# yatpor/bpc_baseline

Hardware: NVIDIA B200
Metric: matched+triangulated scenes/s with the ROI crops of every match (crops/s alongside) (higher is better)
Workload: dtype f64 geometry / u8+f32 crops

## Files before the change

### bpc_baseline_b200/_lib.py

```python
from __future__ import annotations

import ctypes as C
import os

HERE = os.path.dirname(os.path.abspath(__file__))
LIB_PATH = os.environ.get('BPC_LIB') or os.path.join(HERE, 'libbpc_b200.so')

_p = C.c_void_p
_i = C.c_int
_f = C.c_float
_sz = C.c_size_t

SIGNATURES = {
    'bpc_abi_version': (_i, []),
    'bpc_error_string': (C.c_char_p, [_i]),
    'bpc_launch_count': (C.c_ulonglong, []),
    'bpc_fundamental': (_i, [_p, _p, _i, _p, _p]),
    'bpc_cost_tensor': (_i, [_p, _p, _p, _i, _i, _p, _p]),
    'bpc_match_objects': (_i, [_p, _i, _i, _i, _i, _f, _p, _p, _p]),
    'bpc_match_workspace_bytes': (_sz, [_i, _i]),
    'bpc_match_triangulate': (_i, [_p, _p, _p, _p, _i, _i, _f, _i, C.c_double, _p, _p, _p, _p, _p, _p, _p, _sz, _p]),
    'bpc_pack_records_bytes': (_sz, [_i, _i]),
    'bpc_pack_records': (_i, [_p, _p, _p, _p, _p, _p, _i, _i, _i, _p, _p]),
    'bpc_triangulate': (_i, [_p, _p, _i, _p, _p]),
    'bpc_projection': (_i, [_p, _p, _i, _p, _p]),
    'bpc_reprojection_error': (_i, [_p, _p, _p, _i, _p, _p]),
    'bpc_epipolar_error': (_i, [_p, _p, _p, _i, _p, _p]),
    'bpc_epipolar_error_full': (_i, [_p, _p, _i, _p, _p]),
    'bpc_triangulate_views': (_i, [_p, _p, _i, _i, _p, _p]),
    'bpc_box_centers': (_i, [_p, _i, _p, _p]),
    'bpc_detections_from_yolo': (_i, [_p, _p, _p, _p, _i, _i, _f, _i, _p, _p, _p, _p]),
    'bpc_build_rois': (_i, [_p, _p, _p, _p, _i, _i, _i, _p, _p, _p]),
    'bpc_train_rois': (_i, [_p, _p, _p, _p, _i, _i, _i, _p, _p]),
    'bpc_roi_crop_workspace_bytes': (_sz, [_i, _i]),
    'bpc_roi_crop': (_i, [_p, _i, _i, _i, _p, _i, _p, _i, _i, _p, _i, _p, _p, _p, _p, _sz, _p]),
    'bpc_roi_crop_u8': (_i, [_p, _i, _i, _i, _p, _i, _p, _i, _i, _p, _p, _p, _p, _sz, _p]),
    'bpc_roi_crop_bf16': (_i, [_p, _i, _i, _i, _p, _i, _p, _i, _i, _p, _i, _p, _p, _p, _p, _sz, _p]),
    'bpc_normalise_lut': (_i, [_p, _p, _p, _p]),
    'bpc_crops_normalise': (_i, [_p, _p, _i, _i, _i, _p, _p, _p]),
    'bpc_color_jitter': (_i, [_p, _i, _i, _p, _p, _i, _p, _p, _p]),
}

_lib = None
ABI_VERSION = 2


class BpcError(RuntimeError):
    pass


def load():
    global _lib
    if _lib is not None:
        return _lib
    if not os.path.exists(LIB_PATH):
        raise BpcError(f'{LIB_PATH} not found: build it with `python -m bpc_baseline_b200.build` '
                       '(or __graft_entry__.build()); there is no CPU fallback')
    lib = C.CDLL(LIB_PATH)
    for name, (res, args) in SIGNATURES.items():
        fn = getattr(lib, name)
        fn.restype = res
        fn.argtypes = args
    if lib.bpc_abi_version() != ABI_VERSION:
        raise BpcError(f'ABI version mismatch: library {lib.bpc_abi_version()}, binding {ABI_VERSION}')
    _lib = lib
    return lib


def check(code: int, what: str):
    if code != 0:
        msg = load().bpc_error_string(code).decode()
        raise BpcError(f'{what} failed with code {code}: {msg}')


def launch_count() -> int:
    return int(load().bpc_launch_count())
```

### bpc_baseline_b200/batched.py

```python
from __future__ import annotations

import ctypes as C
from dataclasses import dataclass
from typing import Optional, Sequence

import numpy as np
import torch

from . import _lib

MEAN = (0.485, 0.456, 0.406)
STD = (0.229, 0.224, 0.225)


def _chk(t: torch.Tensor, dtype, name: str, ndim: Optional[int] = None):
    if not isinstance(t, torch.Tensor):
        raise TypeError(f'{name}: expected a torch.Tensor, got {type(t).__name__}')
    if not t.is_cuda:
        raise RuntimeError(f'{name}: must be a CUDA tensor (no CPU fallback)')
    if t.dtype != dtype:
        raise RuntimeError(f'{name}: dtype {t.dtype}, expected {dtype}')
    if not t.is_contiguous():
        raise RuntimeError(f'{name}: must be contiguous')
    if ndim is not None and t.dim() != ndim:
# ... 216 lines not shown


def epipolar_error_full(F: torch.Tensor, pts: torch.Tensor) -> torch.Tensor:
    _chk(F, torch.float64, 'F', 4); _chk(pts, torch.float64, 'pts', 3)
    n = F.shape[0]
    if tuple(F.shape) != (n, 3, 3, 3) or tuple(pts.shape) != (n, 3, 2):
        raise RuntimeError('expected F [n,3,3,3] and pts [n,3,2]')
    e = torch.empty((n,), dtype=torch.float64, device=F.device)
    with torch.cuda.device(F.device):
        _lib.check(_lib.load().bpc_epipolar_error_full(_p(F), _p(pts), n, _p(e), _stream(F.device)), 'bpc_epipolar_error_full')
    return e


def triangulate_views(P: torch.Tensor, pts: torch.Tensor) -> torch.Tensor:
    _chk(P, torch.float64, 'P', 4); _chk(pts, torch.float64, 'pts', 3)
    n, V = P.shape[0], P.shape[1]
    if tuple(P.shape) != (n, V, 3, 4) or tuple(pts.shape) != (n, V, 2) or not 2 <= V <= 8:
        raise RuntimeError('expected P [n,V,3,4] and pts [n,V,2] with 2 <= V <= 8')
    X = torch.empty((n, 3), dtype=torch.float64, device=P.device)
    with torch.cuda.device(P.device):
        _lib.check(_lib.load().bpc_triangulate_views(_p(P), _p(pts), n, V, _p(X), _stream(P.device)), 'bpc_triangulate_views')
    return X


def build_rois(boxes: torch.Tensor, idx: torch.Tensor, n: torch.Tensor, image_of_scene: torch.Tensor,
               rois: Optional[torch.Tensor] = None) -> tuple[torch.Tensor, torch.Tensor]:
    _chk(boxes, torch.int32, 'boxes', 4); _chk(idx, torch.int32, 'idx', 3); _chk(n, torch.int32, 'n', 1)
    _chk(image_of_scene, torch.int32, 'image_of_scene', 2)
    S, _, D, _ = boxes.shape
    K = idx.shape[1]
    dev = boxes.device
    if rois is None:
        rois = torch.empty((S * K * 3, 5), dtype=torch.int32, device=dev)
    else:
        _chk(rois, torch.int32, 'rois', 2)
        if rois.shape[0] < S * K * 3 or rois.shape[1] != 5:
            raise RuntimeError('rois must be int32 [>= S*Kmax*3, 5]')
    offs = torch.empty((S + 1,), dtype=torch.int32, device=dev)
    with torch.cuda.device(dev):
        _lib.check(_lib.load().bpc_build_rois(_p(boxes), _p(idx), _p(n), _p(image_of_scene), S, D, K, _p(offs), _p(rois),
                                              _stream(dev)), 'bpc_build_rois')
    return rois, offs


_LUT_CACHE: dict = {}


def normalise_lut(device, mean: Sequence[float] = MEAN, std: Sequence[float] = STD) -> torch.Tensor:
    device = torch.device(device)
    key = (device.index if device.index is not None else torch.cuda.current_device(), tuple(mean), tuple(std))
    if key not in _LUT_CACHE:
        lut = torch.empty((3, 256), dtype=torch.float32, device=device)
        m = (C.c_float * 3)(*[float(np.float32(v)) for v in mean])
        s = (C.c_float * 3)(*[float(np.float32(v)) for v in std])
        with torch.cuda.device(device):
            _lib.check(_lib.load().bpc_normalise_lut(m, s, _p(lut), _stream(device)), 'bpc_normalise_lut')
        _LUT_CACHE[key] = lut
    return _LUT_CACHE[key]


_WS_CACHE: dict = {}
MAX_ROIS_PER_LAUNCH = 32768
MAX_TARGET = 1024
MAX_ROI_WIDTH = 8192


def _crop_workspace(dev, R: int, T: int) -> torch.Tensor:
    need = int(_lib.load().bpc_roi_crop_workspace_bytes(int(R), int(T)))
    key = (dev.index if dev.index is not None else torch.cuda.current_device(), int(torch.cuda.current_stream(dev).cuda_stream))
    ws = _WS_CACHE.get(key)
    if ws is None or ws.numel() < need:
        ws = torch.empty((max(need, 1 << 16),), dtype=torch.uint8, device=dev)
        _WS_CACHE[key] = ws
    return ws


def _chk_status(status, R: int) -> None:
    if status is not None:
        _chk(status, torch.int32, 'status', 1)
        if status.shape[0] < R:
            raise RuntimeError('status must hold one int32 per ROI')


def _crop_args(images, rois, T, fill):
    _chk(images, torch.uint8, 'images', 4); _chk(rois, torch.int32, 'rois', 2)
    B, H, W, ch = images.shape
    if ch != 3 or rois.shape[1] != 5:
        raise RuntimeError('images must be [B,H,W,3] and rois [R,5]')
    if not 1 <= int(T) <= MAX_TARGET:
        raise RuntimeError(f'target size must be in 1..{MAX_TARGET}')
    f = (C.c_uint8 * 3)(*[int(v) for v in fill])
    return B, H, W, rois.shape[0], f


def roi_crop(images: torch.Tensor, rois: torch.Tensor, T: int = 256, fill=(255, 255, 255), swap_rb: bool = True,
             lut: Optional[torch.Tensor] = None, n_rois: Optional[torch.Tensor] = None, roi_first: int = 0,
             out: Optional[torch.Tensor] = None, status: Optional[torch.Tensor] = None) -> torch.Tensor:
    B, H, W, R, f = _crop_args(images, rois, T, fill)
    dev = images.device
    if lut is None:
        lut = normalise_lut(dev)
    _chk_lut(lut, dev)
    if out is None:
        out = torch.empty((R, 3, T, T), dtype=torch.float32, device=dev)
    else:
        _chk(out, torch.float32, 'out', 4)
        if out.shape[0] < R or tuple(out.shape[1:]) != (3, T, T):
            raise RuntimeError('out must be [>=R,3,T,T]')
        _chk_device(out, dev, 'out')
    _chk_status(status, R)
    if n_rois is not None:
        _chk(n_rois, torch.int32, 'n_rois')
    ws = _crop_workspace(dev, min(R, MAX_ROIS_PER_LAUNCH), T)
    with torch.cuda.device(dev):
        for lo in range(0, R, MAX_ROIS_PER_LAUNCH):
            r = min(MAX_ROIS_PER_LAUNCH, R - lo)
            _lib.check(_lib.load().bpc_roi_crop(_p(images), B, H, W, _p(rois[lo:lo + r]), r, _p(n_rois), int(roi_first) + lo, int(T),
                                                f, int(bool(swap_rb)), _p(lut), _p(out[lo:lo + r]),
                                                _p(status[lo:lo + r]) if status is not None else None,
                                                _p(ws), ws.numel(), _stream(dev)), 'bpc_roi_crop')
    return out


def roi_crop_bf16(images: torch.Tensor, rois: torch.Tensor, T: int = 256, fill=(255, 255, 255), swap_rb: bool = True,
                  lut: Optional[torch.Tensor] = None, n_rois: Optional[torch.Tensor] = None, roi_first: int = 0,
                  out: Optional[torch.Tensor] = None, status: Optional[torch.Tensor] = None) -> torch.Tensor:
    B, H, W, R, f = _crop_args(images, rois, T, fill)
    dev = images.device
    if lut is None:
        lut = normalise_lut(dev)
    _chk_lut(lut, dev)
    if out is None:
        out = torch.empty((R, 3, T, T), dtype=torch.bfloat16, device=dev, memory_format=torch.channels_last)
    else:
        if out.dtype != torch.bfloat16 or not out.is_cuda or out.dim() != 4 or out.shape[0] < R or tuple(out.shape[1:]) != (3, T, T) \
                or not out.is_contiguous(memory_format=torch.channels_last):
            raise RuntimeError('out must be a channels_last bfloat16 CUDA tensor [>=R,3,T,T]')
        _chk_device(out, dev, 'out')
    _chk_status(status, R)
    if n_rois is not None:
        _chk(n_rois, torch.int32, 'n_rois')
    ws = _crop_workspace(dev, min(R, MAX_ROIS_PER_LAUNCH), T)
    with torch.cuda.device(dev):
        for lo in range(0, R, MAX_ROIS_PER_LAUNCH):
            r = min(MAX_ROIS_PER_LAUNCH, R - lo)
            _lib.check(_lib.load().bpc_roi_crop_bf16(_p(images), B, H, W, _p(rois[lo:lo + r]), r, _p(n_rois), int(roi_first) + lo, int(T),
                                                     f, int(bool(swap_rb)), _p(lut), out[lo:lo + r].data_ptr(),
                                                     _p(status[lo:lo + r]) if status is not None else None,
                                                     _p(ws), ws.numel(), _stream(dev)), 'bpc_roi_crop_bf16')
    return out


def roi_crop_u8(images: torch.Tensor, rois: torch.Tensor, T: int = 256, fill=(255, 255, 255),
                   n_rois: Optional[torch.Tensor] = None, roi_first: int = 0, out: Optional[torch.Tensor] = None,
                status: Optional[torch.Tensor] = None) -> torch.Tensor:
    B, H, W, R, f = _crop_args(images, rois, T, fill)
    dev = images.device
    if out is None:
        out = torch.empty((R, T, T, 3), dtype=torch.uint8, device=dev)
    else:
        _chk(out, torch.uint8, 'out', 4)
        if out.shape[0] < R or tuple(out.shape[1:]) != (T, T, 3):
            raise RuntimeError('out must be uint8 [>=R,T,T,3]')
        _chk_device(out, dev, 'out')
    _chk_status(status, R)
    if n_rois is not None:
        _chk(n_rois, torch.int32, 'n_rois')
    ws = _crop_workspace(dev, min(R, MAX_ROIS_PER_LAUNCH), T)
    with torch.cuda.device(dev):
        for lo in range(0, R, MAX_ROIS_PER_LAUNCH):
            r = min(MAX_ROIS_PER_LAUNCH, R - lo)
            _lib.check(_lib.load().bpc_roi_crop_u8(_p(images), B, H, W, _p(rois[lo:lo + r]), r, _p(n_rois), int(roi_first) + lo, int(T),
                                                   f, _p(out[lo:lo + r]), _p(status[lo:lo + r]) if status is not None else None,
                                                   _p(ws), ws.numel(), _stream(dev)), 'bpc_roi_crop_u8')
    return out


def crops_normalise(sources: Sequence[torch.Tensor], T: int, swap_rb: bool = True, lut: Optional[torch.Tensor] = None,
                    out: Optional[torch.Tensor] = None, device=None) -> torch.Tensor:
    if not 1 <= len(sources) <= 16:
        raise RuntimeError('1..16 sources')
    for s in sources:
        _chk(s, torch.uint8, 'sources[*]', 4)
        if tuple(s.shape[1:]) != (T, T, 3):
            raise RuntimeError('every source must be uint8 [n,T,T,3]')
    dev = torch.device(device) if device is not None else sources[0].device
    if dev.type == 'cuda' and dev.index is None:
        dev = torch.device('cuda', torch.cuda.current_device())
    if lut is None:
        lut = normalise_lut(dev)
    _chk_lut(lut, dev)
    total = sum(int(s.shape[0]) for s in sources)
    if out is None:
        out = torch.empty((total, 3, T, T), dtype=torch.float32, device=dev)
    else:
        _chk(out, torch.float32, 'out', 4)
        if out.shape[0] < total or tuple(out.shape[1:]) != (3, T, T):
            raise RuntimeError('out must be [>=sum(n_s),3,T,T]')
        _chk_device(out, dev, 'out')
    ptrs = (C.c_void_p * len(sources))(*[s.data_ptr() if s.shape[0] else None for s in sources])
    counts = (C.c_int32 * len(sources))(*[int(s.shape[0]) for s in sources])
    with torch.cuda.device(dev):
        _lib.check(_lib.load().bpc_crops_normalise(ptrs, counts, len(sources), int(T), int(bool(swap_rb)), _p(lut), _p(out),
                                                   _stream(dev)), 'bpc_crops_normalise')
    return out


def color_jitter(canvases: torch.Tensor, order: torch.Tensor, factors: torch.Tensor, swap_rb: bool = False,
                 lut: Optional[torch.Tensor] = None, out: Optional[torch.Tensor] = None) -> torch.Tensor:
    _chk(canvases, torch.uint8, 'canvases', 4); _chk(order, torch.int32, 'order', 2); _chk(factors, torch.float32, 'factors', 2)
    n, T = canvases.shape[0], canvases.shape[1]
    if tuple(canvases.shape[1:]) != (T, T, 3) or tuple(order.shape) != (n, 4) or tuple(factors.shape) != (n, 4):
        raise RuntimeError('expected canvases [n,T,T,3], order [n,4] and factors [n,4]')
    if not 1 <= T <= MAX_TARGET:
        raise RuntimeError(f'target size must be in 1..{MAX_TARGET}')
    dev = canvases.device
    if order.device != dev or factors.device != dev:
        raise RuntimeError('canvases, order and factors must be on the same device')
    if lut is None:
        lut = normalise_lut(dev)
    _chk_lut(lut, dev)
    if out is None:
        out = torch.empty((n, 3, T, T), dtype=torch.float32, device=dev)
    else:
        _chk(out, torch.float32, 'out', 4)
        if out.shape[0] < n or tuple(out.shape[1:]) != (3, T, T):
            raise RuntimeError('out must be [>=n,3,T,T]')
        _chk_device(out, dev, 'out')
    with torch.cuda.device(dev):
        _lib.check(_lib.load().bpc_color_jitter(_p(canvases), n, T, _p(order), _p(factors), int(bool(swap_rb)), _p(lut), _p(out),
                                                _stream(dev)), 'bpc_color_jitter')
    return out


def train_rois(xywh: torch.Tensor, W: int, H: int, image: Optional[torch.Tensor] = None, scale: Optional[torch.Tensor] = None,
               shift: Optional[torch.Tensor] = None) -> torch.Tensor:
    _chk(xywh, torch.int32, 'xywh', 2)
    n = xywh.shape[0]
    if xywh.shape[1] != 4:
        raise RuntimeError('xywh must be [n,4]')
    if image is not None:
        _chk(image, torch.int32, 'image', 1)
    if scale is not None:
        _chk(scale, torch.float64, 'scale', 1)
    if shift is not None:
        _chk(shift, torch.int32, 'shift', 2)
        if scale is None:
            raise RuntimeError('shift needs scale (the reference draws both, data_utils.py:257-263)')
    for t, name in ((image, 'image'), (scale, 'scale'), (shift, 'shift')):
        if t is not None and t.shape[0] != n:
            raise RuntimeError(f'{name}: first dimension must be {n}')
    dev = xywh.device
    rois = torch.empty((n, 5), dtype=torch.int32, device=dev)
    with torch.cuda.device(dev):
        _lib.check(_lib.load().bpc_train_rois(_p(xywh), _p(image), _p(scale), _p(shift), n, int(W), int(H), _p(rois),
                                              _stream(dev)), 'bpc_train_rois')
    return rois
# ... 1 lines not shown
```

### bpc_baseline_b200/csrc/crop.cu

```cuda
#include <mutex>
#include <type_traits>

#include "crop_common.cuh"

namespace bpc {

#ifndef BPC_PREP_THREADS
#define BPC_PREP_THREADS 128
#endif
constexpr int PREP_THREADS = BPC_PREP_THREADS;

__device__ void src_row_records(float2* ysrc, int cap, const RoiGeom& g, int maxtaps, int tid, int* bad) {
    const int hpad = min(cap, ((g.h + STREAM_ROWS - 1) / STREAM_ROWS) * STREAM_ROWS + STREAM_ROWS);
    if (g.h + STREAM_ROWS > cap) *bad = 1;
    for (int s = tid; s < hpad; s += PREP_THREADS) ysrc[s] = make_float2(0.f, 0.f);
    __syncthreads();
    for (int d = tid; d < g.new_h && !*bad; d += PREP_THREADS) {
        int ys, yn, fl; float bf, bm, bl;
        area_taps(d, g.scale_y, g.h, ys, yn, bf, bm, bl, fl);
        const int prev_last = d > 0 ? area_last_tap(d - 1, g.scale_y, g.h) : -1;
        if (yn < 1 || yn > maxtaps || ys < prev_last || ys + yn > g.h) { *bad = 1; break; }
        for (int t = 0; t < yn; ++t) {
            const int s = ys + t;
            const bool shared_first = (t == 0 && s == prev_last);
// ... 774 lines not shown
                        const int32_t* __restrict__ glist, const int32_t* __restrict__ gcount, int T, int nbands,
                        uchar4 fill, int swap_rb, const float* __restrict__ lut_g, float* __restrict__ outf, uint8_t* __restrict__ outb) {
    extern __shared__ __align__(16) unsigned char raw[];
    __shared__ RoiGeom g;
    __shared__ YDesc yd[CROP_BAND];
    __shared__ float lut[OUT_U8 ? 1 : 3 * LUT_STRIDE];
    const int tid = threadIdx.x, nth = blockDim.x;
    const long long items = (long long)(*gcount) * nbands;
    if (blockIdx.x >= items) return;
    if (!OUT_U8)
        for (int e = tid; e < 768; e += nth) lut[(e >> 8) * LUT_STRIDE + (e & 255)] = lut_g[e];
    __syncthreads();
    Out<OUT_U8, BF16> out;
    out_init(out, outf, outb, lut, T, swap_rb, fill);
    for (long long item = blockIdx.x; item < items; item += gridDim.x) {
        const int roi = glist[item / nbands], band = (int)(item % nbands);
        __syncthreads();
        if (tid == 0) g = geom[roi];
        __syncthreads();
        crop_generic_band<OUT_U8, BF16>(raw, yd, out, g, roi, band, images, B, H, W, T, tid, nth);
    }
}

__global__ void bpc_lut_kernel(float m0, float m1, float m2, float s0, float s1, float s2, float* __restrict__ lut) {
    const int t = blockIdx.x * blockDim.x + threadIdx.x;
    if (t >= 768) return;
    const int c = t >> 8, v = t & 255;
    const float mean = c == 0 ? m0 : (c == 1 ? m1 : m2);
    const float sd = c == 0 ? s0 : (c == 1 ? s1 : s2);
    lut[t] = __fdiv_rn(__fsub_rn(__fdiv_rn((float)v, 255.f), mean), sd);
}

static int tensor_maps(const uint8_t* images, int B, int H, int W, bool aligned, TmapSet* out) {
    typedef CUresult (*EncodeFn)(CUtensorMap*, CUtensorMapDataType, cuuint32_t, void*, const cuuint64_t*, const cuuint64_t*,
                                 const cuuint32_t*, const cuuint32_t*, CUtensorMapInterleave, CUtensorMapSwizzle,
                                 CUtensorMapL2promotion, CUtensorMapFloatOOBfill);
    static std::mutex mu;
    static TmapSet cached;
    static const uint8_t* k_images = nullptr;
    static int k_B = 0, k_H = 0, k_W = 0, k_dev = -1;
    static EncodeFn encode = nullptr;
    std::lock_guard<std::mutex> lock(mu);
    if (!aligned) { memset(out, 0, sizeof(TmapSet)); return BPC_OK; }
    int dev = 0;
    cudaGetDevice(&dev);
    if (images == k_images && B == k_B && H == k_H && W == k_W && dev == k_dev) { *out = cached; return BPC_OK; }
    if (!encode) {
        cudaDriverEntryPointQueryResult q;
        void* fnp = nullptr;
        cudaError_t e = cudaGetDriverEntryPoint("cuTensorMapEncodeTiled", &fnp, cudaEnableDefault, &q);
        if (e != cudaSuccess) return (int)e;
        if (q != cudaDriverEntryPointSuccess || !fnp) return (int)cudaErrorNotSupported;
        encode = (EncodeFn)fnp;
    }
    const cuuint64_t gdim[2] = {(cuuint64_t)W * 3 / 4, (cuuint64_t)B * H};
    const cuuint64_t gstride[1] = {(cuuint64_t)W * 3};
    const cuuint32_t estr[2] = {1, 1};
    for (int i = 0; i < N_TMAPS; ++i) {
        const int pitch = i < 13 ? 64 + 32 * i : 512 + 64 * (i - 13);
        const cuuint32_t box[2] = {(cuuint32_t)pitch / 4, (cuuint32_t)tmap_rows(pitch)};
        const CUresult r = encode(&cached.m[i], CU_TENSOR_MAP_DATA_TYPE_UINT32, 2, (void*)images, gdim, gstride, box, estr,
                                  CU_TENSOR_MAP_INTERLEAVE_NONE, CU_TENSOR_MAP_SWIZZLE_NONE, BPC_L2_PROMO,
                                  CU_TENSOR_MAP_FLOAT_OOB_FILL_NONE);
        if (r != CUDA_SUCCESS) { k_images = nullptr; return (int)cudaErrorInvalidValue; }
    }
    for (int i = 0; i < N_TMAPS8; ++i) {
        const int pitch = 64 + 32 * i;
        const cuuint32_t box[2] = {(cuuint32_t)pitch / 4, (cuuint32_t)STREAM_ROWS};
        const CUresult r = encode(&cached.m8[i], CU_TENSOR_MAP_DATA_TYPE_UINT32, 2, (void*)images, gdim, gstride, box, estr,
                                  CU_TENSOR_MAP_INTERLEAVE_NONE, CU_TENSOR_MAP_SWIZZLE_NONE, BPC_L2_PROMO,
                                  CU_TENSOR_MAP_FLOAT_OOB_FILL_NONE);
        if (r != CUDA_SUCCESS) { k_images = nullptr; return (int)cudaErrorInvalidValue; }
    }
    k_images = images; k_B = B; k_H = H; k_W = W; k_dev = dev;
    *out = cached;
    return BPC_OK;
}

static size_t ws_off_xdesc(int R) { return (((size_t)R * sizeof(RoiGeom)) + 15) & ~(size_t)15; }
static size_t ws_off_ydesc(int R, int T) { return ws_off_xdesc(R) + (size_t)R * desc_stride(T) * sizeof(float4); }
static size_t ws_off_count(int R, int T) { return ws_off_ydesc(R, T) + (size_t)R * ydesc_stride(T) * sizeof(float4); }
static size_t crop_workspace_bytes(int R, int T) { return ws_off_count(R, T) + 64 + 2 * (size_t)R * sizeof(int32_t) + 64; }

template <bool OUT_U8, bool BF16 = false>
static int launch_crop(const uint8_t* images, int B, int H, int W, const int32_t* rois, int R, const int32_t* n_rois_dev,
                       int roi_first, int T, const uint8_t* fill, int swap_rb, const float* lut, float* outf, uint8_t* outb,
                       int32_t* status, void* workspace, size_t workspace_bytes, void* stream) {
    if (R < 0 || B < 1 || H < 1 || W < 1 || T < 1 || T > BPC_MAX_TARGET || !fill) return BPC_EINVAL;
    if (R > 0 && (!images || !rois || !workspace || (!OUT_U8 && (!lut || !outf)) || (OUT_U8 && !outb))) return BPC_EINVAL;
    if (((uintptr_t)images & 15) != 0 || ((uintptr_t)workspace & 15) != 0) return BPC_EALIGN;
    if (R == 0) return BPC_OK;
    if (workspace_bytes < crop_workspace_bytes(R, T)) return BPC_EWORKSPACE;
    const int nslot = (T + 31) / 32 + 1;
    if ((long long)R * nslot > 0x7fffffffLL) return BPC_ETOOBIG;
    cudaStream_t st = (cudaStream_t)stream;
    unsigned char* wsb = (unsigned char*)workspace;
    RoiGeom* geom = (RoiGeom*)wsb;
    float4* xdesc = (float4*)(wsb + ws_off_xdesc(R));
    float4* ydesc = (float4*)(wsb + ws_off_ydesc(R, T));
    int32_t* gcount = (int32_t*)(wsb + ws_off_count(R, T));
    int32_t* wcount = gcount + 4;
    int32_t* glist = gcount + 16;
    int32_t* list1 = glist + R;
    cudaError_t e = cudaMemsetAsync(gcount, 0, 64, st);
    if (e != cudaSuccess) return (int)e;
    const bool aligned = ((long long)W * 3) % 16 == 0 && (long long)W * 3 >= TMAP_MAX_PITCH;
    const bool use_cta = aligned && T <= CTA_MAX_T && (long long)W * 3 >= cta_pitch_max(T);
    if (BF16 && !use_cta) return BPC_EUNSUPPORTED;
    bpc_crop_prep_kernel<<<R, PREP_THREADS, 0, st>>>(images, B, H, W, rois, R, n_rois_dev, roi_first, T, (aligned ? 1 : 0) | (use_cta ? 2 : 0), geom, xdesc, ydesc,
                                            glist, gcount, status, use_cta ? list1 : nullptr);
    BPC_LAUNCH_CHECK();
    const uchar4 f4 = make_uchar4(fill[0], fill[1], fill[2], 0);
    if (use_cta) {
        const int rc = crop_cta_launch(OUT_U8 ? 1 : (BF16 ? 2 : 0), images, B, H, W, geom, xdesc, ydesc, list1, gcount, R, T, f4, swap_rb, lut,
                                       outf, outb, st);
        if (rc != BPC_OK) return rc;
    }
    if (!use_cta) {
        typedef void (*WarpFn)(const uint8_t*, int, int, int, const RoiGeom*, const float4*, const float4*, int32_t*, int, int, int,
                               uchar4, int, const float*, float*, uint8_t*, const TmapSet, const int32_t*);
        TmapSet tmaps;
        const int terr = tensor_maps(images, B, H, W, aligned, &tmaps);
        if (terr != BPC_OK) return terr;
        WarpFn fn;
        const bool sw = swap_rb != 0;
#define BPC_PICK(TTV)                                                                                                  \
    (aligned ? (sw ? bpc_crop_warp_kernel<OUT_U8, TTV, true, true> : bpc_crop_warp_kernel<OUT_U8, TTV, true, false>)   \
             : (sw ? bpc_crop_warp_kernel<OUT_U8, TTV, false, true> : bpc_crop_warp_kernel<OUT_U8, TTV, false, false>))
        if (OUT_U8) fn = aligned ? bpc_crop_warp_kernel<OUT_U8, 0, true, false> : bpc_crop_warp_kernel<OUT_U8, 0, false, false>;
        else if (T == 224) fn = BPC_PICK(224);
        else if (T == 256) fn = BPC_PICK(256);
        else fn = BPC_PICK(0);
#undef BPC_PICK
        e = cudaFuncSetAttribute(fn, cudaFuncAttributeMaxDynamicSharedMemorySize, WARPK_SMEM);
        if (e != cudaSuccess) return (int)e;
        const int cta_threads = 256;
        const long long nitems = (long long)R * nslot;
        const long long want = (nitems + WARPK_WARPS - 1) / WARPK_WARPS;
        int dev = 0, sms = 148, per_sm = 3;
        cudaGetDevice(&dev);
        cudaDeviceGetAttribute(&sms, cudaDevAttrMultiProcessorCount, dev);
        if (cudaOccupancyMaxActiveBlocksPerMultiprocessor(&per_sm, fn, cta_threads, WARPK_SMEM) != cudaSuccess || per_sm < 1) per_sm = 1;
        const long long slots = (long long)sms * per_sm;
        const int grid = (int)(want < slots ? want : slots);
        fn<<<grid, cta_threads, WARPK_SMEM, st>>>(images, B, H, W, geom, xdesc, ydesc, wcount, R, T, nslot, f4, swap_rb, lut, outf, outb, tmaps, use_cta ? list1 : nullptr);
        BPC_LAUNCH_CHECK();
    }
    const int nbands = (T + CROP_BAND - 1) / CROP_BAND;
    const long long max_items = (long long)R * nbands;
    const int grid = (int)(max_items < 148 * 2 ? max_items : 148 * 2);
    const int threads = ((T + 31) / 32) * 32;
    if (threads <= 256) {
        e = cudaFuncSetAttribute(bpc_crop_generic_kernel<OUT_U8, 256, BF16>, cudaFuncAttributeMaxDynamicSharedMemorySize, CROP_RAW_BYTES);
        if (e != cudaSuccess) return (int)e;
        bpc_crop_generic_kernel<OUT_U8, 256, BF16><<<grid, threads, CROP_RAW_BYTES, st>>>(images, B, H, W, geom, glist, gcount, T, nbands, f4,
                                                                                   swap_rb, lut, outf, outb);
    } else {
        e = cudaFuncSetAttribute(bpc_crop_generic_kernel<OUT_U8, 1024, BF16>, cudaFuncAttributeMaxDynamicSharedMemorySize, CROP_RAW_BYTES);
        if (e != cudaSuccess) return (int)e;
        bpc_crop_generic_kernel<OUT_U8, 1024, BF16><<<grid, threads, CROP_RAW_BYTES, st>>>(images, B, H, W, geom, glist, gcount, T, nbands, f4,
                                                                                    swap_rb, lut, outf, outb);
    }
    BPC_LAUNCH_CHECK();
    return BPC_OK;
}

}

using namespace bpc;

extern "C" size_t bpc_roi_crop_workspace_bytes(int R, int T) { return (R < 0 || T < 1 || T > BPC_MAX_TARGET) ? 0 : crop_workspace_bytes(R, T); }

extern "C" int bpc_roi_crop(const uint8_t* images, int B, int H, int W, const int32_t* rois, int R,
                            const int32_t* n_rois_dev, int roi_first, int T, const uint8_t* fill, int swap_rb,
                            const float* lut, float* out, int32_t* status, void* workspace, size_t workspace_bytes,
                            void* stream) {
    if (((uintptr_t)out & 15) != 0) return BPC_EALIGN;
    return launch_crop<false>(images, B, H, W, rois, R, n_rois_dev, roi_first, T, fill, swap_rb, lut, out, nullptr, status,
                              workspace, workspace_bytes, stream);
}

extern "C" int bpc_roi_crop_bf16(const uint8_t* images, int B, int H, int W, const int32_t* rois, int R,
                                 const int32_t* n_rois_dev, int roi_first, int T, const uint8_t* fill, int swap_rb,
                                 const float* lut, void* out, int32_t* status, void* workspace, size_t workspace_bytes,
                                 void* stream) {
    if (((uintptr_t)out & 15) != 0) return BPC_EALIGN;
    return launch_crop<false, true>(images, B, H, W, rois, R, n_rois_dev, roi_first, T, fill, swap_rb, lut, (float*)out, nullptr, status,
                                    workspace, workspace_bytes, stream);
}

extern "C" int bpc_roi_crop_u8(const uint8_t* images, int B, int H, int W, const int32_t* rois, int R,
                               const int32_t* n_rois_dev, int roi_first, int T, const uint8_t* fill, uint8_t* out,
                               int32_t* status, void* workspace, size_t workspace_bytes, void* stream) {
    return launch_crop<true>(images, B, H, W, rois, R, n_rois_dev, roi_first, T, fill, 0, nullptr, nullptr, out, status,
                             workspace, workspace_bytes, stream);
}

extern "C" int bpc_normalise_lut(const float* mean, const float* std_, float* lut, void* stream) {
    if (!mean || !std_ || !lut) return BPC_EINVAL;
    bpc_lut_kernel<<<3, 256, 0, (cudaStream_t)stream>>>(mean[0], mean[1], mean[2], std_[0], std_[1], std_[2], lut);
    BPC_LAUNCH_CHECK();
    return BPC_OK;
}
```

### bpc_baseline_b200/pipeline.py

```python
from __future__ import annotations

from typing import Callable, Optional

import numpy as np
import torch

from . import batched
from ._host import nvtx_range


class MatchCropPipeline:
    def __init__(self, S: int, Dmax: int, *, T: int = 224, chunk_rois: int = 16384, threshold=30,
                 swap_rb: bool = True, fill=(255, 255, 255), device='cuda', want_reproj: bool = True,
                 reproj_thresh: Optional[float] = None, crops: Optional[torch.Tensor] = None,
                 crop_dtype: torch.dtype = torch.float32):
        self.S, self.D, self.T = int(S), int(Dmax), int(T)
        self.device = torch.device(device)
        self.threshold = threshold
        self.swap_rb, self.fill, self.want_reproj, self.reproj_thresh = swap_rb, tuple(fill), want_reproj, reproj_thresh
        self.cap = self.S * self.D * 3
        self.chunk = max(1, min(int(chunk_rois), self.cap))
        dev = self.device
        self.rois = torch.zeros((self.cap, 5), dtype=torch.int32, device=dev)
        if crop_dtype not in (torch.float32, torch.bfloat16):
            raise RuntimeError('crop_dtype must be torch.float32 or torch.bfloat16')
        self.crop_dtype = crop_dtype
        if crop_dtype == torch.bfloat16:
            if crops is not None:
                raise RuntimeError('a caller-owned chunk buffer is float32 only')
            self.crops = torch.empty((self.chunk, 3, self.T, self.T), dtype=torch.bfloat16, device=dev, memory_format=torch.channels_last)
        elif crops is not None:
            if crops.dtype != torch.float32 or not crops.is_contiguous() or crops.numel() < self.chunk * 3 * self.T * self.T:
                raise RuntimeError('crops must be a contiguous float32 buffer of at least chunk_rois * 3 * T * T elements')
            self.crops = crops.view(-1)[:self.chunk * 3 * self.T * self.T].view(self.chunk, 3, self.T, self.T)
        else:
            self.crops = torch.empty((self.chunk, 3, self.T, self.T), dtype=torch.float32, device=dev)
        self.status = torch.zeros((self.cap,), dtype=torch.int32, device=dev)
        self.lut = batched.normalise_lut(dev)
        self._host = None
        self.last_crop_launches = 0

    def run_device(self, Ks, RTs, centers, counts, boxes, images, image_of_scene,
                   consumer: Optional[Callable[[torch.Tensor, int], None]] = None,
                   n_rois_host: Optional[int] = None, events=None):
        with nvtx_range('bpc.match'):
            res = batched.match_triangulate(Ks, RTs, centers, counts, self.threshold, want_reproj=self.want_reproj,
                                            reproj_thresh=self.reproj_thresh)
        with nvtx_range('bpc.build_rois'):
            rois, offs = batched.build_rois(boxes, res.idx, res.n, image_of_scene, rois=self.rois)
        total = offs[self.S:self.S + 1]
        if events is not None:
            events[0].record()
            events[1].record()
        upto = self.cap if n_rois_host is None else min(self.cap, int(n_rois_host))
        launches = 0
        for first in range(0, upto, self.chunk):
            r = min(self.chunk, self.cap - first)
            with nvtx_range('bpc.crop_chunk'):
                crop = batched.roi_crop_bf16 if self.crop_dtype == torch.bfloat16 else batched.roi_crop
                out = crop(images, rois[first:first + r], T=self.T, fill=self.fill, swap_rb=self.swap_rb,
                           lut=self.lut, n_rois=total, roi_first=first, out=self.crops, status=self.status[first:first + r])
            launches += 1
            if consumer is not None:
                consumer(out[:r], first)
        if events is not None:
            events[2].record()
        self.last_crop_launches = launches
        return res, offs

    def _alloc_host(self, images_shape):
        S, D, dev = self.S, self.D, self.device
        pin = lambda shape, dt: torch.empty(shape, dtype=dt).pin_memory()
        h = {
            'Ks': pin((S, 3, 3, 3), torch.float32), 'RTs': pin((S, 3, 4, 4), torch.float64),
            'boxes': pin((S, 3, D, 4), torch.int32), 'counts': pin((S, 3), torch.int32),
            'image_of_scene': pin((S, 3), torch.int32), 'images': pin(tuple(images_shape), torch.uint8),
            'idx': pin((S, D, 3), torch.int32), 'n': pin((S,), torch.int32), 'cost': pin((S, D), torch.float32),
            'X': pin((S, D, 3), torch.float64), 'n_rois': pin((1,), torch.int32),
        }
        d = {k: torch.empty(h[k].shape, dtype=h[k].dtype, device=dev)
             for k in ('Ks', 'RTs', 'boxes', 'counts', 'image_of_scene', 'images')}
        self._host = (h, d)

    def host_buffers(self, images_shape):
        if self._host is None or tuple(self._host[0]['images'].shape) != tuple(images_shape):
            self._alloc_host(images_shape)
        return self._host[0]

    def run_host(self, consumer=None, n_rois_host=None):
        h, d = self._host
        for k in d:
            d[k].copy_(h[k], non_blocking=True)
        centers = batched.box_centers(d['boxes'])
        res, offs = self.run_device(d['Ks'], d['RTs'], centers, d['counts'], d['boxes'], d['images'],
                                    d['image_of_scene'], consumer=consumer, n_rois_host=n_rois_host)
        h['idx'].copy_(res.idx, non_blocking=True)
        h['n'].copy_(res.n, non_blocking=True)
        h['cost'].copy_(res.cost, non_blocking=True)
        h['X'].copy_(res.X, non_blocking=True)
        h['n_rois'].copy_(offs[self.S:self.S + 1], non_blocking=True)
        torch.cuda.current_stream(self.device).synchronize()
        return h

    def run_host_stream(self, steps: int, refill: Optional[Callable[[dict, int], None]] = None,
                        on_result: Optional[Callable[[dict, int], None]] = None, consumer=None):
        h, d = self._host
        dev = self.device
        if not hasattr(self, '_stream_state'):
            d2 = {k: torch.empty_like(v) for k, v in d.items()}
            res_keys = ('idx', 'n', 'cost', 'X', 'n_rois')
            h2 = {k: torch.empty_like(h[k]).pin_memory() for k in res_keys}
            self._stream_state = {'d': (d, d2), 'hres': ({k: h[k] for k in res_keys}, h2),
                                  'copy': torch.cuda.Stream(device=dev)}
        st = self._stream_state
        main = torch.cuda.current_stream(dev)
        up_done = [torch.cuda.Event(), torch.cuda.Event()]
        free = [torch.cuda.Event(), torch.cuda.Event()]
        res_done = [torch.cuda.Event(), torch.cuda.Event()]
        host_read = [torch.cuda.Event(), torch.cuda.Event()]

        def upload(k):
            j = k & 1
            if refill is not None:
                if k >= 1:
                    host_read[(k - 1) & 1].synchronize()
                refill(h, k)
            with torch.cuda.stream(st['copy']):
                if k >= 2:
                    st['copy'].wait_event(free[j])
                for key, t in st['d'][j].items():
                    t.copy_(h[key], non_blocking=True)
                up_done[j].record(st['copy'])
                host_read[j].record(st['copy'])

        upload(0)
        for k in range(steps):
            j = k & 1
            if k + 1 < steps:
                upload(k + 1)
            main.wait_event(up_done[j])
            dj = st['d'][j]
            centers = batched.box_centers(dj['boxes'])
            res, offs = self.run_device(dj['Ks'], dj['RTs'], centers, dj['counts'], dj['boxes'], dj['images'],
                                        dj['image_of_scene'], consumer=consumer)
            free[j].record(main)
            if k >= 2:
                res_done[j].synchronize()
            hr = st['hres'][j]
            hr['idx'].copy_(res.idx, non_blocking=True)
            hr['n'].copy_(res.n, non_blocking=True)
# ... 28 lines not shown
```

### include/bpc_b200.h

```cpp
#ifndef BPC_B200_H
#define BPC_B200_H

#include <stddef.h>
#include <stdint.h>

#ifdef __cplusplus
extern "C" {
#endif

#define BPC_ABI_VERSION 2

enum {
    BPC_OK = 0,
    BPC_EINVAL = -1,
    BPC_EALIGN = -2,
    BPC_EWORKSPACE = -3,
    BPC_ETOOBIG = -4,
    BPC_EUNSUPPORTED = -5
};

#define BPC_N_INFEASIBLE (-1)
#define BPC_N_OVERFLOW (-2)

#define BPC_MAX_DET 2048
#define BPC_MAX_ROI_WIDTH 8192
#define BPC_MAX_TARGET 1024

int bpc_abi_version(void);
const char* bpc_error_string(int code);

int bpc_fundamental(const float* Ks, const double* RTs, int S, double* F, void* stream);

int bpc_cost_tensor(const double* F, const double* centers, const int32_t* counts, int S, int Dmax,
                    float* cost, void* stream);

int bpc_match_objects(const float* cost, int S, int N, int M, int P, float threshold,
                      int32_t* idx, int32_t* n, void* stream);

size_t bpc_match_workspace_bytes(int S, int Dmax);
int bpc_match_triangulate(const float* Ks, const double* RTs, const double* centers, const int32_t* counts,
                          int S, int Dmax, float threshold, int has_reproj_thresh, double reproj_thresh,
                          int32_t* idx, int32_t* n, float* cost, double* X, double* reproj, double* F,
                          void* workspace, size_t workspace_bytes, void* stream);

size_t bpc_pack_records_bytes(int S, int Kmax);
int bpc_pack_records(const int32_t* idx, const int32_t* n, const float* cost, const double* X, const double* reproj,
                     const int32_t* scene_offset, int offset_div, int S, int Kmax, void* buf, void* stream);

int bpc_triangulate(const double* P, const double* pts, int n, double* X, void* stream);
int bpc_projection(const float* K, const double* RT, int n, double* P, void* stream);
int bpc_reprojection_error(const double* P, const double* X, const double* pts, int n, double* err, void* stream);

int bpc_epipolar_error(const double* F, const double* pt1, const double* pt2, int n, double* e, void* stream);
int bpc_epipolar_error_full(const double* F, const double* pts, int n, double* e, void* stream);
int bpc_triangulate_views(const double* P, const double* pts, int n, int V, double* X, void* stream);

int bpc_box_centers(const int32_t* boxes, int count, double* centers, void* stream);

int bpc_detections_from_yolo(const float* xyxy, const float* conf, const float* cls, const int32_t* nraw, int SC, int Nraw,
                             float conf_thresh, int Dmax, int32_t* boxes, double* centers, int32_t* counts, void* stream);

int bpc_build_rois(const int32_t* boxes, const int32_t* idx, const int32_t* n, const int32_t* image_of_scene,
                   int S, int Dmax, int Kmax, int32_t* scene_offset, int32_t* rois, void* stream);

int bpc_train_rois(const int32_t* xywh, const int32_t* image, const double* scale, const int32_t* shift, int n,
                   int W, int H, int32_t* rois, void* stream);

size_t bpc_roi_crop_workspace_bytes(int R, int T);
int bpc_roi_crop(const uint8_t* images, int B, int H, int W, const int32_t* rois, int R,
                 const int32_t* n_rois_dev, int roi_first, int T, const uint8_t* fill, int swap_rb,
                 const float* lut, float* out, int32_t* status,
                 void* workspace, size_t workspace_bytes, void* stream);
int bpc_roi_crop_u8(const uint8_t* images, int B, int H, int W, const int32_t* rois, int R,
                    const int32_t* n_rois_dev, int roi_first, int T, const uint8_t* fill,
                    uint8_t* out, int32_t* status,
                    void* workspace, size_t workspace_bytes, void* stream);
int bpc_roi_crop_bf16(const uint8_t* images, int B, int H, int W, const int32_t* rois, int R,
                      const int32_t* n_rois_dev, int roi_first, int T, const uint8_t* fill, int swap_rb,
                      const float* lut, void* out, int32_t* status,
                      void* workspace, size_t workspace_bytes, void* stream);
int bpc_normalise_lut(const float* mean_host3, const float* std_host3, float* lut, void* stream);

int bpc_crops_normalise(const uint8_t* const* srcs, const int32_t* counts, int n_src, int T, int swap_rb,
                        const float* lut, float* out, void* stream);

int bpc_color_jitter(const uint8_t* in, int n, int T, const int32_t* order, const float* factors, int swap_rb,
                     const float* lut, float* out, void* stream);

unsigned long long bpc_launch_count(void);

#ifdef __cplusplus
}
#endif
#endif
```

Before: 115,500.

## Split ROI crop into prepare/run and overlap prep on a side stream

The crop launcher is split into a prepare step (memset plus per-ROI geometry and descriptor kernel) and a run step (the actual crop kernels), each exposed through the C ABI. The pipeline double-buffers two workspaces and issues prepare for the next part on a secondary stream while the main stream runs the current crop, synchronised with events. The goal is to hide the prep kernel latency behind crop execution. In exchange it adds extra event and stream synchronisation plus more Python launch overhead per part, and the consumer is now called on chunk boundaries.

```diff
diff --git a/bpc_baseline_b200/_lib.py b/bpc_baseline_b200/_lib.py
--- a/bpc_baseline_b200/_lib.py
+++ b/bpc_baseline_b200/_lib.py
@@ -36,6 +36,10 @@
     'bpc_roi_crop': (_i, [_p, _i, _i, _i, _p, _i, _p, _i, _i, _p, _i, _p, _p, _p, _p, _sz, _p]),
     'bpc_roi_crop_u8': (_i, [_p, _i, _i, _i, _p, _i, _p, _i, _i, _p, _p, _p, _p, _sz, _p]),
     'bpc_roi_crop_bf16': (_i, [_p, _i, _i, _i, _p, _i, _p, _i, _i, _p, _i, _p, _p, _p, _p, _sz, _p]),
+    'bpc_roi_crop_prepare': (_i, [_p, _i, _i, _i, _p, _i, _p, _i, _i, _p, _p, _sz, _p]),
+    'bpc_roi_crop_run': (_i, [_p, _i, _i, _i, _i, _i, _p, _i, _p, _p, _p, _sz, _p]),
+    'bpc_roi_crop_run_bf16': (_i, [_p, _i, _i, _i, _i, _i, _p, _i, _p, _p, _p, _sz, _p]),
+    'bpc_roi_crop_run_u8': (_i, [_p, _i, _i, _i, _i, _i, _p, _p, _p, _sz, _p]),
     'bpc_normalise_lut': (_i, [_p, _p, _p, _p]),
     'bpc_crops_normalise': (_i, [_p, _p, _i, _i, _i, _p, _p, _p]),
     'bpc_color_jitter': (_i, [_p, _i, _i, _p, _p, _i, _p, _p, _p]),
diff --git a/bpc_baseline_b200/batched.py b/bpc_baseline_b200/batched.py
--- a/bpc_baseline_b200/batched.py
+++ b/bpc_baseline_b200/batched.py
@@ -322,14 +322,22 @@
             raise RuntimeError('status must hold one int32 per ROI')
 
 
-def _crop_args(images, rois, T, fill):
-    _chk(images, torch.uint8, 'images', 4); _chk(rois, torch.int32, 'rois', 2)
+def _image_args(images, T, fill):
+    _chk(images, torch.uint8, 'images', 4)
     B, H, W, ch = images.shape
-    if ch != 3 or rois.shape[1] != 5:
-        raise RuntimeError('images must be [B,H,W,3] and rois [R,5]')
+    if ch != 3:
+        raise RuntimeError('images must be [B,H,W,3]')
     if not 1 <= int(T) <= MAX_TARGET:
         raise RuntimeError(f'target size must be in 1..{MAX_TARGET}')
     f = (C.c_uint8 * 3)(*[int(v) for v in fill])
+    return B, H, W, f
+
+
+def _crop_args(images, rois, T, fill):
+    _chk(images, torch.uint8, 'images', 4); _chk(rois, torch.int32, 'rois', 2)
+    if images.shape[3] != 3 or rois.shape[1] != 5:
+        raise RuntimeError('images must be [B,H,W,3] and rois [R,5]')
+    B, H, W, f = _image_args(images, T, fill)
     return B, H, W, rois.shape[0], f
 
 
@@ -413,6 +421,66 @@
             _lib.check(_lib.load().bpc_roi_crop_u8(_p(images), B, H, W, _p(rois[lo:lo + r]), r, _p(n_rois), int(roi_first) + lo, int(T),
                                                    f, _p(out[lo:lo + r]), _p(status[lo:lo + r]) if status is not None else None,
                                                    _p(ws), ws.numel(), _stream(dev)), 'bpc_roi_crop_u8')
+    return out
+
+
+def crop_workspace(dev, R: int, T: int) -> torch.Tensor:
+    if not 0 <= int(R) <= MAX_ROIS_PER_LAUNCH or not 1 <= int(T) <= MAX_TARGET:
+        raise RuntimeError(f'R must be in 0..{MAX_ROIS_PER_LAUNCH} and T in 1..{MAX_TARGET}')
+    return torch.empty((max(int(_lib.load().bpc_roi_crop_workspace_bytes(int(R), int(T))), 1 << 16),), dtype=torch.uint8, device=dev)
+
+
+def _chk_workspace(workspace: torch.Tensor, dev: torch.device, R: int, T: int) -> None:
+    _chk(workspace, torch.uint8, 'workspace', 1)
+    _chk_device(workspace, dev, 'workspace')
+    if R > MAX_ROIS_PER_LAUNCH:
+        raise RuntimeError(f'at most {MAX_ROIS_PER_LAUNCH} ROIs per prepared workspace')
+
+
+def roi_crop_prepare(images: torch.Tensor, rois: torch.Tensor, workspace: torch.Tensor, T: int = 256,
+                     n_rois: Optional[torch.Tensor] = None, roi_first: int = 0, status: Optional[torch.Tensor] = None) -> None:
+    B, H, W, R, _ = _crop_args(images, rois, T, (0, 0, 0))
+    dev = images.device
+    _chk_device(rois, dev, 'rois')
+    _chk_workspace(workspace, dev, R, T)
+    _chk_status(status, R)
+    if n_rois is not None:
+        _chk(n_rois, torch.int32, 'n_rois')
+    with torch.cuda.device(dev):
+        _lib.check(_lib.load().bpc_roi_crop_prepare(_p(images), B, H, W, _p(rois), R, _p(n_rois), int(roi_first), int(T), _p(status),
+                                                    _p(workspace), workspace.numel(), _stream(dev)), 'bpc_roi_crop_prepare')
+
+
+def roi_crop_run(images: torch.Tensor, R: int, workspace: torch.Tensor, T: int = 256, fill=(255, 255, 255), swap_rb: bool = True,
+                 lut: Optional[torch.Tensor] = None, out: Optional[torch.Tensor] = None,
+                 dtype: torch.dtype = torch.float32) -> torch.Tensor:
+    B, H, W, f = _image_args(images, T, fill)
+    R = int(R)
+    dev = images.device
+    _chk_workspace(workspace, dev, R, T)
+    if lut is None:
+        lut = normalise_lut(dev)
+    _chk_lut(lut, dev)
+    if dtype == torch.float32:
+        if out is None:
+            out = torch.empty((R, 3, T, T), dtype=torch.float32, device=dev)
+        _chk(out, torch.float32, 'out', 4)
+        if out.shape[0] < R or tuple(out.shape[1:]) != (3, T, T):
+            raise RuntimeError('out must be [>=R,3,T,T]')
+        fn, name = _lib.load().bpc_roi_crop_run, 'bpc_roi_crop_run'
+    elif dtype == torch.bfloat16:
+        if out is None:
+            out = torch.empty((R, 3, T, T), dtype=torch.bfloat16, device=dev, memory_format=torch.channels_last)
+        if out.dtype != torch.bfloat16 or not out.is_cuda or out.dim() != 4 or out.shape[0] < R or tuple(out.shape[1:]) != (3, T, T) \
+                or not out.is_contiguous(memory_format=torch.channels_last):
+            raise RuntimeError('out must be a channels_last bfloat16 CUDA tensor [>=R,3,T,T]')
+        fn, name = _lib.load().bpc_roi_crop_run_bf16, 'bpc_roi_crop_run_bf16'
+    else:
+        raise RuntimeError('dtype must be torch.float32 or torch.bfloat16')
+    _chk_device(out, dev, 'out')
+    with torch.cuda.device(dev):
+        _lib.check(fn(_p(images), B, H, W, R, int(T), f, int(bool(swap_rb)), _p(lut), out.data_ptr(), _p(workspace), workspace.numel(),
+                      _stream(dev)), name)
     return out
 
 
diff --git a/bpc_baseline_b200/csrc/crop.cu b/bpc_baseline_b200/csrc/crop.cu
--- a/bpc_baseline_b200/csrc/crop.cu
+++ b/bpc_baseline_b200/csrc/crop.cu
@@ -880,34 +880,60 @@
 static size_t ws_off_count(int R, int T) { return ws_off_ydesc(R, T) + (size_t)R * ydesc_stride(T) * sizeof(float4); }
 static size_t crop_workspace_bytes(int R, int T) { return ws_off_count(R, T) + 64 + 2 * (size_t)R * sizeof(int32_t) + 64; }
 
-template <bool OUT_U8, bool BF16 = false>
-static int launch_crop(const uint8_t* images, int B, int H, int W, const int32_t* rois, int R, const int32_t* n_rois_dev,
-                       int roi_first, int T, const uint8_t* fill, int swap_rb, const float* lut, float* outf, uint8_t* outb,
-                       int32_t* status, void* workspace, size_t workspace_bytes, void* stream) {
-    if (R < 0 || B < 1 || H < 1 || W < 1 || T < 1 || T > BPC_MAX_TARGET || !fill) return BPC_EINVAL;
-    if (R > 0 && (!images || !rois || !workspace || (!OUT_U8 && (!lut || !outf)) || (OUT_U8 && !outb))) return BPC_EINVAL;
+struct CropWs {
+    RoiGeom* geom; float4* xdesc; float4* ydesc; int32_t* gcount; int32_t* wcount; int32_t* glist; int32_t* list1;
+    CropWs(void* workspace, int R, int T) {
+        unsigned char* wsb = (unsigned char*)workspace;
+        geom = (RoiGeom*)wsb;
+        xdesc = (float4*)(wsb + ws_off_xdesc(R));
+        ydesc = (float4*)(wsb + ws_off_ydesc(R, T));
+        gcount = (int32_t*)(wsb + ws_off_count(R, T));
+        wcount = gcount + 4;
+        glist = gcount + 16;
+        list1 = glist + R;
+    }
+};
+
+static bool crop_aligned(int W) { return ((long long)W * 3) % 16 == 0 && (long long)W * 3 >= TMAP_MAX_PITCH; }
+static bool crop_use_cta(int W, int T) { return crop_aligned(W) && T <= CTA_MAX_T && (long long)W * 3 >= cta_pitch_max(T); }
+
+static int crop_check(const uint8_t* images, int B, int H, int W, int R, int T, bool ptrs, int out_mode, const uint8_t* fill,
+                      void* workspace, size_t workspace_bytes) {
+    if (R < 0 || B < 1 || H < 1 || W < 1 || T < 1 || T > BPC_MAX_TARGET || (out_mode >= 0 && !fill)) return BPC_EINVAL;
+    if (R > 0 && (!images || !workspace || !ptrs)) return BPC_EINVAL;
     if (((uintptr_t)images & 15) != 0 || ((uintptr_t)workspace & 15) != 0) return BPC_EALIGN;
     if (R == 0) return BPC_OK;
     if (workspace_bytes < crop_workspace_bytes(R, T)) return BPC_EWORKSPACE;
+    if ((long long)R * ((T + 31) / 32 + 1) > 0x7fffffffLL) return BPC_ETOOBIG;
+    if (out_mode == 2 && !crop_use_cta(W, T)) return BPC_EUNSUPPORTED;
+    return BPC_OK;
+}
+
+template <bool OUT_U8, bool BF16>
+static bool crop_out_ok(const float* lut, const float* outf, const uint8_t* outb) { return OUT_U8 ? outb != nullptr : (lut && outf); }
+
+static int crop_prepare(const uint8_t* images, int B, int H, int W, const int32_t* rois, int R, const int32_t* n_rois_dev, int roi_first,
+                        int T, int32_t* status, void* workspace, cudaStream_t st) {
+    CropWs ws(workspace, R, T);
+    cudaError_t e = cudaMemsetAsync(ws.gcount, 0, 64, st);
+    if (e != cudaSuccess) return (int)e;
+    const bool aligned = crop_aligned(W), use_cta = crop_use_cta(W, T);
+    bpc_crop_prep_kernel<<<R, PREP_THREADS, 0, st>>>(images, B, H, W, rois, R, n_rois_dev, roi_first, T, (aligned ? 1 : 0) | (use_cta ? 2 : 0),
+                                                     ws.geom, ws.xdesc, ws.ydesc, ws.glist, ws.gcount, status, use_cta ? ws.list1 : nullptr);
+    BPC_LAUNCH_CHECK();
+    return BPC_OK;
+}
+
+template <bool OUT_U8, bool BF16 = false>
+static int crop_run(const uint8_t* images, int B, int H, int W, int R, int T, const uint8_t* fill, int swap_rb, const float* lut,
+                    float* outf, uint8_t* outb, void* workspace, cudaStream_t st) {
+    const CropWs ws(workspace, R, T);
+    const RoiGeom* geom = ws.geom;
+    const float4 *xdesc = ws.xdesc, *ydesc = ws.ydesc;
+    int32_t *gcount = ws.gcount, *wcount = ws.wcount, *glist = ws.glist, *list1 = ws.list1;
     const int nslot = (T + 31) / 32 + 1;
-    if ((long long)R * nslot > 0x7fffffffLL) return BPC_ETOOBIG;
-    cudaStream_t st = (cudaStream_t)stream;
-    unsigned char* wsb = (unsigned char*)workspace;
-    RoiGeom* geom = (RoiGeom*)wsb;
-    float4* xdesc = (float4*)(wsb + ws_off_xdesc(R));
-    float4* ydesc = (float4*)(wsb + ws_off_ydesc(R, T));
-    int32_t* gcount = (int32_t*)(wsb + ws_off_count(R, T));
-    int32_t* wcount = gcount + 4;
-    int32_t* glist = gcount + 16;
-    int32_t* list1 = glist + R;
-    cudaError_t e = cudaMemsetAsync(gcount, 0, 64, st);
-    if (e != cudaSuccess) return (int)e;
-    const bool aligned = ((long long)W * 3) % 16 == 0 && (long long)W * 3 >= TMAP_MAX_PITCH;
-    const bool use_cta = aligned && T <= CTA_MAX_T && (long long)W * 3 >= cta_pitch_max(T);
-    if (BF16 && !use_cta) return BPC_EUNSUPPORTED;
-    bpc_crop_prep_kernel<<<R, PREP_THREADS, 0, st>>>(images, B, H, W, rois, R, n_rois_dev, roi_first, T, (aligned ? 1 : 0) | (use_cta ? 2 : 0), geom, xdesc, ydesc,
-                                            glist, gcount, status, use_cta ? list1 : nullptr);
-    BPC_LAUNCH_CHECK();
+    const bool aligned = crop_aligned(W), use_cta = crop_use_cta(W, T);
+    cudaError_t e;
     const uchar4 f4 = make_uchar4(fill[0], fill[1], fill[2], 0);
     if (use_cta) {
         const int rc = crop_cta_launch(OUT_U8 ? 1 : (BF16 ? 2 : 0), images, B, H, W, geom, xdesc, ydesc, list1, gcount, R, T, f4, swap_rb, lut,
@@ -963,6 +989,28 @@
     return BPC_OK;
 }
 
+template <bool OUT_U8, bool BF16 = false>
+static int launch_crop(const uint8_t* images, int B, int H, int W, const int32_t* rois, int R, const int32_t* n_rois_dev,
+                       int roi_first, int T, const uint8_t* fill, int swap_rb, const float* lut, float* outf, uint8_t* outb,
+                       int32_t* status, void* workspace, size_t workspace_bytes, void* stream) {
+    int rc = crop_check(images, B, H, W, R, T, rois && crop_out_ok<OUT_U8, BF16>(lut, outf, outb), OUT_U8 ? 1 : (BF16 ? 2 : 0), fill,
+                        workspace, workspace_bytes);
+    if (rc != BPC_OK || R == 0) return rc;
+    cudaStream_t st = (cudaStream_t)stream;
+    rc = crop_prepare(images, B, H, W, rois, R, n_rois_dev, roi_first, T, status, workspace, st);
+    if (rc != BPC_OK) return rc;
+    return crop_run<OUT_U8, BF16>(images, B, H, W, R, T, fill, swap_rb, lut, outf, outb, workspace, st);
+}
+
+template <bool OUT_U8, bool BF16 = false>
+static int run_prepared(const uint8_t* images, int B, int H, int W, int R, int T, const uint8_t* fill, int swap_rb, const float* lut,
+                        float* outf, uint8_t* outb, void* workspace, size_t workspace_bytes, void* stream) {
+    const int rc = crop_check(images, B, H, W, R, T, crop_out_ok<OUT_U8, BF16>(lut, outf, outb), OUT_U8 ? 1 : (BF16 ? 2 : 0), fill,
+                              workspace, workspace_bytes);
+    if (rc != BPC_OK || R == 0) return rc;
+    return crop_run<OUT_U8, BF16>(images, B, H, W, R, T, fill, swap_rb, lut, outf, outb, workspace, (cudaStream_t)stream);
+}
+
 }
 
 using namespace bpc;
@@ -978,6 +1026,31 @@
                               workspace, workspace_bytes, stream);
 }
 
+extern "C" int bpc_roi_crop_prepare(const uint8_t* images, int B, int H, int W, const int32_t* rois, int R,
+                                    const int32_t* n_rois_dev, int roi_first, int T, int32_t* status, void* workspace,
+                                    size_t workspace_bytes, void* stream) {
+    const int rc = crop_check(images, B, H, W, R, T, rois != nullptr, -1, nullptr, workspace, workspace_bytes);
+    if (rc != BPC_OK || R == 0) return rc;
+    return crop_prepare(images, B, H, W, rois, R, n_rois_dev, roi_first, T, status, workspace, (cudaStream_t)stream);
+}
+
+extern "C" int bpc_roi_crop_run(const uint8_t* images, int B, int H, int W, int R, int T, const uint8_t* fill, int swap_rb,
+                                const float* lut, float* out, void* workspace, size_t workspace_bytes, void* stream) {
+    if (((uintptr_t)out & 15) != 0) return BPC_EALIGN;
+    return run_prepared<false>(images, B, H, W, R, T, fill, swap_rb, lut, out, nullptr, workspace, workspace_bytes, stream);
+}
+
+extern "C" int bpc_roi_crop_run_bf16(const uint8_t* images, int B, int H, int W, int R, int T, const uint8_t* fill, int swap_rb,
+                                     const float* lut, void* out, void* workspace, size_t workspace_bytes, void* stream) {
+    if (((uintptr_t)out & 15) != 0) return BPC_EALIGN;
+    return run_prepared<false, true>(images, B, H, W, R, T, fill, swap_rb, lut, (float*)out, nullptr, workspace, workspace_bytes, stream);
+}
+
+extern "C" int bpc_roi_crop_run_u8(const uint8_t* images, int B, int H, int W, int R, int T, const uint8_t* fill, uint8_t* out,
+                                   void* workspace, size_t workspace_bytes, void* stream) {
+    return run_prepared<true>(images, B, H, W, R, T, fill, 0, nullptr, nullptr, out, workspace, workspace_bytes, stream);
+}
+
 extern "C" int bpc_roi_crop_bf16(const uint8_t* images, int B, int H, int W, const int32_t* rois, int R,
                                  const int32_t* n_rois_dev, int roi_first, int T, const uint8_t* fill, int swap_rb,
                                  const float* lut, void* out, int32_t* status, void* workspace, size_t workspace_bytes,
diff --git a/bpc_baseline_b200/pipeline.py b/bpc_baseline_b200/pipeline.py
--- a/bpc_baseline_b200/pipeline.py
+++ b/bpc_baseline_b200/pipeline.py
@@ -37,6 +37,13 @@
             self.crops = torch.empty((self.chunk, 3, self.T, self.T), dtype=torch.float32, device=dev)
         self.status = torch.zeros((self.cap,), dtype=torch.int32, device=dev)
         self.lut = batched.normalise_lut(dev)
+        self.part = min(self.chunk, batched.MAX_ROIS_PER_LAUNCH)
+        self._ws = [batched.crop_workspace(dev, self.part, self.T) for _ in range(2)]
+        with torch.cuda.device(dev):
+            self._setup = torch.cuda.Stream(device=dev, priority=0)
+        self._prepared = [torch.cuda.Event(), torch.cuda.Event()]
+        self._ran = [torch.cuda.Event(), torch.cuda.Event()]
+        self._rois_ready = torch.cuda.Event()
         self._host = None
         self.last_crop_launches = 0
 
@@ -49,23 +56,43 @@
         with nvtx_range('bpc.build_rois'):
             rois, offs = batched.build_rois(boxes, res.idx, res.n, image_of_scene, rois=self.rois)
         total = offs[self.S:self.S + 1]
+        main = torch.cuda.current_stream(self.device)
         if events is not None:
-            events[0].record()
-            events[1].record()
+            events[0].record(main)
+            events[1].record(main)
         upto = self.cap if n_rois_host is None else min(self.cap, int(n_rois_host))
-        launches = 0
-        for first in range(0, upto, self.chunk):
-            r = min(self.chunk, self.cap - first)
+        parts = [(p, min(self.part, first + r - p), p - first)
+                 for first in range(0, upto, self.chunk) for r in (min(self.chunk, self.cap - first),)
+                 for p in range(first, first + r, self.part)]
+        self._rois_ready.record(main)
+        self._setup.wait_event(self._rois_ready)
+
+        def prepare(k):
+            first, r, _ = parts[k]
+            j = k & 1
+            with torch.cuda.stream(self._setup), nvtx_range('bpc.crop_prepare'):
+                if k >= 2:
+                    self._setup.wait_event(self._ran[j])
+                batched.roi_crop_prepare(images, rois[first:first + r], self._ws[j], T=self.T, n_rois=total, roi_first=first,
+                                         status=self.status[first:first + r])
+                self._prepared[j].record(self._setup)
+
+        if parts:
+            prepare(0)
+        for k, (first, r, row) in enumerate(parts):
+            j = k & 1
+            if k + 1 < len(parts):
+                prepare(k + 1)
+            main.wait_event(self._prepared[j])
             with nvtx_range('bpc.crop_chunk'):
-                crop = batched.roi_crop_bf16 if self.crop_dtype == torch.bfloat16 else batched.roi_crop
-                out = crop(images, rois[first:first + r], T=self.T, fill=self.fill, swap_rb=self.swap_rb,
-                           lut=self.lut, n_rois=total, roi_first=first, out=self.crops, status=self.status[first:first + r])
-            launches += 1
-            if consumer is not None:
-                consumer(out[:r], first)
+                batched.roi_crop_run(images, r, self._ws[j], T=self.T, fill=self.fill, swap_rb=self.swap_rb, lut=self.lut,
+                                     out=self.crops[row:], dtype=self.crop_dtype)
+            self._ran[j].record(main)
+            if consumer is not None and (k + 1 == len(parts) or parts[k + 1][2] == 0):
+                consumer(self.crops[:row + r], first - row)
         if events is not None:
-            events[2].record()
-        self.last_crop_launches = launches
+            events[2].record(main)
+        self.last_crop_launches = len(range(0, upto, self.chunk))
         return res, offs
 
     def _alloc_host(self, images_shape):
diff --git a/include/bpc_b200.h b/include/bpc_b200.h
--- a/include/bpc_b200.h
+++ b/include/bpc_b200.h
@@ -79,6 +79,15 @@
                       const int32_t* n_rois_dev, int roi_first, int T, const uint8_t* fill, int swap_rb,
                       const float* lut, void* out, int32_t* status,
                       void* workspace, size_t workspace_bytes, void* stream);
+int bpc_roi_crop_prepare(const uint8_t* images, int B, int H, int W, const int32_t* rois, int R,
+                         const int32_t* n_rois_dev, int roi_first, int T, int32_t* status,
+                         void* workspace, size_t workspace_bytes, void* stream);
+int bpc_roi_crop_run(const uint8_t* images, int B, int H, int W, int R, int T, const uint8_t* fill, int swap_rb,
+                     const float* lut, float* out, void* workspace, size_t workspace_bytes, void* stream);
+int bpc_roi_crop_run_bf16(const uint8_t* images, int B, int H, int W, int R, int T, const uint8_t* fill, int swap_rb,
+                          const float* lut, void* out, void* workspace, size_t workspace_bytes, void* stream);
+int bpc_roi_crop_run_u8(const uint8_t* images, int B, int H, int W, int R, int T, const uint8_t* fill, uint8_t* out,
+                        void* workspace, size_t workspace_bytes, void* stream);
 int bpc_normalise_lut(const float* mean_host3, const float* std_host3, float* lut, void* stream);
 
 int bpc_crops_normalise(const uint8_t* const* srcs, const int32_t* counts, int n_src, int T, int swap_rb,
```

After: 117,100, median of 6. 1.4% higher.
